# ibejarano/Pynama

Measured on AMD Instinct MI355X. Metric: assembled element-DOFs/sec + CG iterations/sec, 10M-DOF Poisson, 1/2/4/8 MI355X, higher is better.
Workload: dtype f64

## Files before the change

### pynama_amd/csrc/pyn_assemble_lattice.hip

```cpp
#include "pyn_internal.h"
#include "pyn_q1_hex.h"
#include "pyn_lattice.h"

namespace {


__device__ __forceinline__ double lat_affine_inv(const double* __restrict__ S, const double (&E)[3][3], double (&Ji)[3][3]) {
  double J[3][3];
#pragma unroll
  for (int d = 0; d < 3; ++d)
#pragma unroll
    for (int x = 0; x < 3; ++x) J[d][x] = fma(S[d * 3 + 2], E[2][x], fma(S[d * 3 + 1], E[1][x], S[d * 3] * E[0][x]));
  const double c00 = J[1][1] * J[2][2] - J[1][2] * J[2][1];
  const double c01 = J[1][2] * J[2][0] - J[1][0] * J[2][2];
  const double c02 = J[1][0] * J[2][1] - J[1][1] * J[2][0];
  const double det = J[0][0] * c00 + J[0][1] * c01 + J[0][2] * c02;
  const double r = 1.0 / det;
  Ji[0][0] = c00 * r;
  Ji[0][1] = (J[0][2] * J[2][1] - J[0][1] * J[2][2]) * r;
  Ji[0][2] = (J[0][1] * J[1][2] - J[0][2] * J[1][1]) * r;
  Ji[1][0] = c01 * r;
  Ji[1][1] = (J[0][0] * J[2][2] - J[0][2] * J[2][0]) * r;
  Ji[1][2] = (J[0][2] * J[1][0] - J[0][0] * J[1][2]) * r;
  Ji[2][0] = c02 * r;
  Ji[2][1] = (J[0][1] * J[2][0] - J[0][0] * J[2][1]) * r;
  Ji[2][2] = (J[0][0] * J[1][1] - J[0][1] * J[1][0]) * r;
  return det;
}

__device__ __forceinline__ void lat_affine_corners(const LatArgs& T, int n00, int gl, double (&C4)[4][3]) {
  const int nx = T.nx;
  const double* q0 = T.xyz + (int64_t)(lat_plane(T, gl) + n00) * 3;
  const double* qz = T.xyz + (int64_t)(lat_plane(T, gl + 1) + n00) * 3;
  if (T.ablate == 32) {
#pragma unroll
    for (int d = 0; d < 4; ++d)
#pragma unroll
      for (int x = 0; x < 3; ++x) C4[d][x] = (d == x + 1) ? 0.005 : 0.0;
    return;
  }
#pragma unroll
  for (int x = 0; x < 3; ++x) {
    C4[0][x] = q0[x];
    C4[1][x] = q0[3 + x];
    C4[2][x] = q0[3 * nx + x];
    C4[3][x] = qz[x];
  }
}
__device__ __forceinline__ double lat_affine_geom_from(const double* __restrict__ S, const double (&C4)[4][3], double (&Ji)[3][3]) {
  double E[3][3];
#pragma unroll
  for (int d = 0; d < 3; ++d)
#pragma unroll
    for (int x = 0; x < 3; ++x) E[d][x] = C4[d + 1][x] - C4[0][x];
  return lat_affine_inv(S, E, Ji);
}
__device__ __forceinline__ double lat_affine_geom(const LatArgs& T, const double* __restrict__ S, int n00, int gl, double (&Ji)[3][3]) {
  double C4[4][3];
  lat_affine_corners(T, n00, gl, C4);
  return lat_affine_geom_from(S, C4, Ji);
}

__device__ __forceinline__ void lat_affine_L_from(const double (&Ji)[3][3], const double det, double (&L)[36]) {
  double Q[6];
  {
    constexpr int RS[6][2] = {{0, 0}, {1, 1}, {2, 2}, {0, 1}, {0, 2}, {1, 2}};
#pragma unroll
    for (int u = 0; u < 6; ++u) {
      const int a = RS[u][0], b = RS[u][1];
      Q[u] = det * (Ji[0][a] * Ji[0][b] + Ji[1][a] * Ji[1][b] + Ji[2][a] * Ji[2][b]);
    }
  }
  {
    double D[3][3], M[3][2];
#pragma unroll
    for (int u = 0; u < 3; ++u) {
      const double qd = Q[u] * (1.0 / 72.0), qm = Q[3 + u] * (1.0 / 72.0);
      D[u][0] = 4.0 * qd;
      D[u][1] = 8.0 * qd;
      D[u][2] = 16.0 * qd;
      M[u][0] = 12.0 * qm;
      M[u][1] = 24.0 * qm;
    }
    int idx = 0;
#pragma unroll
// ... 687 lines not shown
      unsigned char f[NJ];
#pragma unroll
      for (int j = 0; j < NJ; ++j) {
        const int i = tid + 256 * j;
        const int qx = i % MT::BX, qy = (i / MT::BX) % MT::BY, qz = i / (MT::BX * MT::BY);
        const int x = x0 - 1 + qx, y = y0 - 1 + qy, pl = T.p_own0 + z0 - 1 + qz;
        v[j] = 0.0;
        f[j] = 0;
        if (i < MT::NB && x >= 0 && x < nx && y >= 0 && y < ny && pl >= 0 && pl < T.npl) {
          const int64_t node = lat_plane(T, pl) + y * nx + x;
          f[j] = T.bcmask ? T.bcmask[node] : 0;
          v[j] = xin[node];
        }
      }
#pragma unroll
      for (int j = 0; j < NJ; ++j) {
        const int i = tid + 256 * j;
        if (i < MT::NB) {
          xs[i] = f[j] ? 0.0 : v[j];
          nbc[i] = f[j];
        }
      }
    }
    for (int i = tid; i < MT::NR; i += 256) acc[i] = 0.0;
    __syncthreads();
    {
      const int gx = x0 - 1 + lx, gy = y0 - 1 + ly;
      const bool col_ok = gx >= 0 && gx < nx - 1 && gy >= 0 && gy < ny - 1;
      const int n00 = gy * nx + gx;
      double xb[4], carry[4] = {0.0, 0.0, 0.0, 0.0};
#pragma unroll
      for (int c = 0; c < 4; ++c) xb[c] = xs[boff[c]];
#pragma nounroll
      for (int lz = 0; lz <= TZ; ++lz) {
        const int gl = T.p_own0 + z0 - 1 + lz;
        double xe[8], ye[8];
#pragma unroll
        for (int c = 0; c < 4; ++c) {
          xe[c] = xb[c];
          xe[TOP[c]] = xs[(lz + 1) * (MT::BX * MT::BY) + boff[c]];
        }
        if (col_ok && gl >= 0 && gl < T.npl - 1 && T.ablate != 1) {
          double Ji[3][3];
          const double det = lat_affine_geom(T, S, n00, gl, Ji);
          lat_affine_apply(Ji, det, xe, ye);
        } else {
#pragma unroll
          for (int a = 0; a < 8; ++a) ye[a] = 0.0;
        }
        if (lz >= 1) {
#pragma unroll
          for (int c = 0; c < 4; ++c)
            if (rok[c]) atomicAdd(&acc[(lz - 1) * 225 + roff[c]], carry[c] + ye[c]);
        }
#pragma unroll
        for (int c = 0; c < 4; ++c) {
          carry[c] = ye[TOP[c]];
          xb[c] = xe[TOP[c]];
        }
      }
    }
    __syncthreads();
    for (int s = tid; s < MT::NR; s += 256) {
      const int rx = s % 15, ry = (s / 15) % 15, rz = s / 225;
      const int x = x0 + rx, y = y0 + ry, zo = z0 + rz;
      if (x >= nx || y >= ny || zo >= T.n_own) continue;
      const int64_t node = lat_plane(T, T.p_own0 + zo) + y * nx + x;
      const int bi = ((rz + 1) * MT::BY + ry + 1) * MT::BX + rx + 1;
      const double xv = nbc[bi] ? xin[node] : xs[bi];
      const double yv = nbc[bi] ? xv : acc[s];
      yout[node] = yv;
      if (DOT) dot = fma(yv, xv, dot);
    }
    __syncthreads();
  }
  if (DOT) {
    for (int o = 32; o > 0; o >>= 1) dot += __shfl_xor(dot, o, 64);
    if ((tid & 63) == 0) smd[tid >> 6] = dot;
    __syncthreads();
    if (tid == 0) part[blockIdx.x] = smd[0] + smd[1] + smd[2] + smd[3];
  }
}

struct KleLatArgs {
  LatArgs L;
  double alpha_d, alpha_w;
  const double *wr, *hrsr, *Hr, *hcoor;
  const double* Lel = nullptr;
  int64_t ne = 0;
};

__device__ __forceinline__ double jac_inverse(const double* __restrict__ hc, const double (&X)[8][3], double (&Ji)[3][3]) {
  double J[3][3];
#pragma unroll
  for (int d = 0; d < 3; ++d)
#pragma unroll
    for (int x = 0; x < 3; ++x) {
      double s = 0.0;
#pragma unroll
      for (int c = 0; c < 8; ++c) s = fma(hc[d * 8 + c], X[c][x], s);
      J[d][x] = s;
    }
  const double c00 = J[1][1] * J[2][2] - J[1][2] * J[2][1];
  const double c01 = J[1][2] * J[2][0] - J[1][0] * J[2][2];
  const double c02 = J[1][0] * J[2][1] - J[1][1] * J[2][0];
  const double det = J[0][0] * c00 + J[0][1] * c01 + J[0][2] * c02;
  const double r = 1.0 / det;
  Ji[0][0] = c00 * r;
  Ji[0][1] = (J[0][2] * J[2][1] - J[0][1] * J[2][2]) * r;
  Ji[0][2] = (J[0][1] * J[1][2] - J[0][2] * J[1][1]) * r;
  Ji[1][0] = c01 * r;
  Ji[1][1] = (J[0][0] * J[2][2] - J[0][2] * J[2][0]) * r;
  Ji[1][2] = (J[0][2] * J[1][0] - J[0][0] * J[1][2]) * r;
  Ji[2][0] = c02 * r;
  Ji[2][1] = (J[0][1] * J[2][0] - J[0][0] * J[2][1]) * r;
  Ji[2][2] = (J[0][0] * J[1][1] - J[0][1] * J[1][0]) * r;
  return det;
}

__device__ __forceinline__ void kle_reduced_apply(const KleLatArgs& T, const double (&Ji)[3][3], double det, const double (&xe)[8][3],
                                                  double (&ye)[8][3]) {
  const double* __restrict__ hr = T.hrsr;
  const double cr = T.wr[0] * det;
  const double caw = cr * T.alpha_w, cad = cr * T.alpha_d;
  double Gr[3][8];
#pragma unroll
  for (int d = 0; d < 3; ++d)
#pragma unroll
    for (int a = 0; a < 8; ++a) Gr[d][a] = fma(Ji[d][2], hr[16 + a], fma(Ji[d][1], hr[8 + a], Ji[d][0] * hr[a]));
  double D[3][3];
#pragma unroll
  for (int d = 0; d < 3; ++d)
#pragma unroll
    for (int q = 0; q < 3; ++q) {
      double sacc = 0.0;
#pragma unroll
      for (int b = 0; b < 8; ++b) sacc = fma(Gr[d][b], xe[b][q], sacc);
      D[d][q] = sacc;
    }
  const double tr = cad * (D[0][0] + D[1][1] + D[2][2]);
  double W[3][3];
#pragma unroll
  for (int d = 0; d < 3; ++d)
#pragma unroll
    for (int pp = 0; pp < 3; ++pp) W[d][pp] = d == pp ? tr : caw * (D[d][pp] - D[pp][d]);
#pragma unroll
  for (int a = 0; a < 8; ++a)
#pragma unroll
    for (int pp = 0; pp < 3; ++pp)
      ye[a][pp] = fma(Gr[2][a], W[2][pp], fma(Gr[1][a], W[1][pp], fma(Gr[0][a], W[0][pp], ye[a][pp])));
}

template <int TX, int TY, int TZ, bool AFF, bool DOT>
__global__ void __launch_bounds__(256) lattice_matfree_kle_kernel(KleLatArgs K, const double* __restrict__ xin, double* __restrict__ yout,
                                                                   const int* __restrict__ flag, double* __restrict__ part, int n_tiles) {
  using MT = MfTile<TX, TY, TZ>;
  extern __shared__ __align__(16) double lds[];
  __shared__ double smd[4];
  if (flag && flag[0]) return;
  const LatArgs& T = K.L;
  double* xs = lds;
  double* acc = xs + MT::NB * 3;
  unsigned char* nbc = reinterpret_cast<unsigned char*>(acc + MT::NR * 3);
  const int tid = threadIdx.x;
  const int nx = T.nx, ny = T.ny;
  const double* __restrict__ S = AFF ? T.q.aff + 248 : nullptr;
// ... 911 lines not shown
  }
  PYN_HIP(hipGetLastError());
  return PYN_OK;
}

int pyn_assemble_kle_lattice(pyn_ctx* c, const AsmRequest& rq, const AsmKnobs& k, const AsmPlan& P) {
  KleLatArgs T;
  lat_fill(c, k, T.L);
  kle_fill(c, T, rq.alpha_d, rq.alpha_w);
  T.L.rhs_clean = rq.rhs_clean ? 1 : 0;
  T.L.rcrow = rq.rcrow;
  if (P.kle_general) return launch_kle_lattice<3, 3, 3, true>(c, T, rq.K, rq.Krhs, rq.Rw);
  switch (P.shape) {
    case 1: return launch_kle_lattice<6, 2, 2, false>(c, T, rq.K, rq.Krhs, rq.Rw);
    case 2: return launch_kle_lattice<3, 3, 2, false>(c, T, rq.K, rq.Krhs, rq.Rw);
    case 3: return launch_kle_lattice<4, 3, 3, false>(c, T, rq.K, rq.Krhs, rq.Rw);
    case 4: return launch_kle_lattice<5, 2, 2, false>(c, T, rq.K, rq.Krhs, rq.Rw);
    default: return launch_kle_lattice<3, 3, 3, false>(c, T, rq.K, rq.Krhs, rq.Rw);
  }
}

int pyn_assemble_lattice(pyn_ctx* c, AsmRequest& rq, const AsmKnobs& k, const AsmPlan& P) {
  LatArgs T;
  lat_fill(c, k, T);
  T.A = rq.K;
  T.Arhs = P.krhs_pending ? nullptr : rq.Krhs;
  T.rhs_clean = rq.rhs_clean ? 1 : 0;
  T.rcrow = rq.rcrow;
  T.dinv = P.dinv ? rq.dinv : nullptr;
  rq.dinv_written = T.dinv != nullptr;
  const bool tiles_closed = P.kind == AK_LATTICE && P.k_closed;
  if (tiles_closed && !k.no_lattice_axes && k.lattice_ablate != 32) {
    PYN_TRY(pyn_lattice_axes_ensure(c, k));
    if (c->lat.rect == 1) {
      T.axX = c->lat.d_axes;
      T.axY = T.axX + lat_axis_slots(T.nx);
      T.axZ = T.axY + lat_axis_slots(T.ny);
    }
  }
  PYN_CHECK(!k.lattice_axes_require || T.axX,
            "PYNAMA_LATTICE_AXES_REQUIRE: the axis-table variant of the lattice tile kernel does not apply (%s)",
            !tiles_closed ? "not the parallelepiped tile kernel" : k.no_lattice_axes || k.lattice_ablate == 32 ? "switched off"
                                                                                                              : "mesh not rectilinear");
  int rows_nl = k.lattice_rows_lines == 2 ? 2 : 1;
  while (rows_nl > 1 && lat_rows_lds(T.nx, rows_nl) > 64 * 1024) rows_nl /= 2;
  const char* no_rows = !tiles_closed                                                                ? "not the parallelepiped tile kernel"
                        : k.no_lattice_rows                                                          ? "switched off"
                        : k.lattice_tile >= 0                                                        ? "PYNAMA_LATTICE_TILE asks for a tile shape"
                        : k.lattice_ablate != 0                                                      ? "PYNAMA_LATTICE_ABLATE is set"
                        : k.no_lattice_axes || k.lattice_axes_require || k.no_lattice_tilebc         ? "a switch of the tile kernel's variants is set"
                        : rq.rcrow                                                                   ? "compact Arhs"
                        : c->lat.rect != 1                                                           ? "mesh not rectilinear"
                        : lat_rows_lds(T.nx, rows_nl) > 64 * 1024                                            ? "x-lines too long for the LDS staging"
                                                                                                     : nullptr;
  PYN_CHECK(!k.lattice_rows_require || !no_rows, "PYNAMA_LATTICE_ROWS_REQUIRE: the rows kernel of rectilinear lattices does not apply (%s)",
            no_rows);
  if (!no_rows) {
    if (rows_nl == 2) return launch_lattice_rows<2, 256>(c, T);
    switch (k.lattice_rows_threads) {
      case 128: return launch_lattice_rows<1, 128>(c, T);
      case 512: return launch_lattice_rows<1, 512>(c, T);
      default: return launch_lattice_rows<1, 256>(c, T);
    }
  }
  if (k.lattice_ablate == 64) T.bcmask = nullptr;
  if (P.kind == AK_MARCH) return pyn_assemble_lattice_march(c, k, &T, P.shape);
  const bool affine = P.k_closed, tilebc = !k.no_lattice_tilebc;
  switch (P.shape) {
    case 1: return launch_lattice<7, 7, 7>(c, T, affine, tilebc);
    case 2: return launch_lattice<6, 6, 6>(c, T, affine, tilebc);
    case 3: return launch_lattice<8, 6, 6>(c, T, affine, tilebc);
    case 4: return launch_lattice<7, 6, 6>(c, T, affine, tilebc);
    case 5: return launch_lattice<6, 6, 4>(c, T, affine, tilebc);
    case 6: return launch_lattice<6, 5, 5>(c, T, affine, tilebc);
    case 7: return launch_lattice<7, 4, 4>(c, T, affine, tilebc);
    case 8: return launch_lattice<14, 3, 3>(c, T, affine, tilebc);
    case 9: return launch_lattice<7, 5, 5>(c, T, affine, tilebc);
    default: return launch_lattice<7, 5, 4>(c, T, affine, tilebc);
  }
}


static int mf_select_layers(LatArgs& T, int ntz, int zsel) {
  const int lo = T.p_own0 > 0 ? 1 : 0, hi = T.p_own0 + T.n_own < T.npl ? 1 : 0;
  T.bz0 = 0;
  T.bzs = 1;
  if (zsel == 0) return ntz;
  const int n_int = std::max(0, ntz - lo - hi);
  if (zsel == 1) {
    T.bz0 = lo;
    return n_int;
  }
  if (n_int == 0) return ntz;
  if (lo && hi) {
    T.bzs = ntz - 1;
    return 2;
  }
  T.bz0 = hi ? ntz - 1 : 0;
  return lo + hi;
}

struct MfLaunch {
  int zsel = 0, part_off = 0, max_grid = PYN_MAX_PARTIALS;
  hipStream_t st = nullptr;
};

template <int TX, int TY, int TZ>
static int launch_matfree(pyn_ctx* c, LatArgs& T, bool affine, const double* x, double* y, bool dot, const MfLaunch& L, int* grid_out) {
  using MT = MfTile<TX, TY, TZ>;
  T.ntx = (T.nx + TX - 1) / TX;
  T.nty = (T.ny + TY - 1) / TY;
  const int n_tiles = T.ntx * T.nty * mf_select_layers(T, (T.n_own + TZ - 1) / TZ, L.zsel);
  const int grid = std::min(n_tiles, L.max_grid);
  if (grid_out) *grid_out = grid;
  if (grid == 0) return PYN_OK;
  const int* flag = dot ? c->d_flag : nullptr;
  double* part = dot ? c->d_part + L.part_off : nullptr;
  hipStream_t s = L.st;
  if (affine) {
    if (dot)
      lattice_matfree_laplace_kernel<TX, TY, TZ, true, true><<<grid, 256, MT::BYTES, s>>>(T, x, y, flag, part, n_tiles);
    else
      lattice_matfree_laplace_kernel<TX, TY, TZ, true, false><<<grid, 256, MT::BYTES, s>>>(T, x, y, flag, part, n_tiles);
  } else {
    if (dot)
      lattice_matfree_laplace_kernel<TX, TY, TZ, false, true><<<grid, 256, MT::BYTES, s>>>(T, x, y, flag, part, n_tiles);
    else
      lattice_matfree_laplace_kernel<TX, TY, TZ, false, false><<<grid, 256, MT::BYTES, s>>>(T, x, y, flag, part, n_tiles);
  }
  PYN_HIP(hipGetLastError());
  return PYN_OK;
}

template <int TZ>
static int launch_matfree_march(pyn_ctx* c, LatArgs& T, const double* x, double* y, bool dot, const MfLaunch& L, int* grid_out) {
  using MT = MfTile<15, 15, TZ>;
  T.ntx = (T.nx + 14) / 15;
  T.nty = (T.ny + 14) / 15;
  const int n_tiles = T.ntx * T.nty * mf_select_layers(T, (T.n_own + TZ - 1) / TZ, L.zsel);
  const int grid = std::min(n_tiles, L.max_grid);
  if (grid_out) *grid_out = grid;
  if (grid == 0) return PYN_OK;
  if (dot)
    lattice_matfree_laplace_march_kernel<TZ, true><<<grid, 256, MT::BYTES, L.st>>>(T, x, y, c->d_flag, c->d_part + L.part_off, n_tiles);
  else
    lattice_matfree_laplace_march_kernel<TZ, false><<<grid, 256, MT::BYTES, L.st>>>(T, x, y, nullptr, nullptr, n_tiles);
  PYN_HIP(hipGetLastError());
  return PYN_OK;
}

static bool q1_matfree_supported(const pyn_ctx* c) {
  return c->lat.valid && c->dim == 3 && c->nn == 8 && c->quad[0].ngp == 8;
}

static int matfree_laplace_launch(pyn_ctx* c, const double* x, double* y, bool dot, const MfLaunch& L, int* grid_out) {
  PYN_CHECK(q1_matfree_supported(c), "matrix-free operator: needs a Q1 hexahedral mesh with structured topology and the "
                                               "full-rule tables");
  PYN_CHECK(c->mf_set[PYN_MATFREE_LAPLACE], "matrix-free Laplacian: pyn_matfree_set first");
  LatArgs T;
  int mesh_aff = 0;
  PYN_TRY(lat_fill_args(c, T, &mesh_aff));
  T.bcmask = c->mf_mask[PYN_MATFREE_LAPLACE];
  const bool affine = mesh_aff == 1 && T.q.aff != nullptr && c->aff_standard;
  const char* tl = getenv("PYNAMA_MATFREE_TILE");
  const int sel = tl ? atoi(tl) : (affine ? 6 : 0);
  if (affine && sel >= 6) {
    switch (sel) {
      case 7: return launch_matfree_march<4>(c, T, x, y, dot, L, grid_out);
      case 8: return launch_matfree_march<6>(c, T, x, y, dot, L, grid_out);
      case 9: return launch_matfree_march<12>(c, T, x, y, dot, L, grid_out);
      default: return launch_matfree_march<8>(c, T, x, y, dot, L, grid_out);
    }
  }
  switch (sel) {
    case 1: PYN_TRY((launch_matfree<16, 8, 4>(c, T, affine, x, y, dot, L, grid_out))); break;
    case 2: PYN_TRY((launch_matfree<8, 8, 8>(c, T, affine, x, y, dot, L, grid_out))); break;
    case 3: PYN_TRY((launch_matfree<16, 4, 4>(c, T, affine, x, y, dot, L, grid_out))); break;
    case 4: PYN_TRY((launch_matfree<32, 4, 4>(c, T, affine, x, y, dot, L, grid_out))); break;
    case 5: PYN_TRY((launch_matfree<12, 6, 6>(c, T, affine, x, y, dot, L, grid_out))); break;
    default: PYN_TRY((launch_matfree<16, 8, 8>(c, T, affine, x, y, dot, L, grid_out))); break;
  }
  return PYN_OK;
}

template <int TX, int TY, int TZ>
static int launch_matfree_kle(pyn_ctx* c, KleLatArgs& K, bool affine, const double* x, double* y, bool dot, const MfLaunch& L, int* grid_out) {
  using MT = MfTile<TX, TY, TZ>;
  LatArgs& T = K.L;
  T.ntx = (T.nx + TX - 1) / TX;
  T.nty = (T.ny + TY - 1) / TY;
  const int n_tiles = T.ntx * T.nty * mf_select_layers(T, (T.n_own + TZ - 1) / TZ, L.zsel);
  const int grid = std::min(n_tiles, L.max_grid);
  if (grid_out) *grid_out = grid;
  if (grid == 0) return PYN_OK;
  const size_t lds = (size_t)(MT::NB + MT::NR) * 3 * sizeof(double) + ((MT::NB + 7) & ~7);
  const int* flag = dot ? c->d_flag : nullptr;
  double* part = dot ? c->d_part + L.part_off : nullptr;
  hipStream_t s = L.st;
  if (affine) {
    if (dot)
      lattice_matfree_kle_kernel<TX, TY, TZ, true, true><<<grid, 256, lds, s>>>(K, x, y, flag, part, n_tiles);
    else
      lattice_matfree_kle_kernel<TX, TY, TZ, true, false><<<grid, 256, lds, s>>>(K, x, y, flag, part, n_tiles);
  } else {
    if (dot)
      lattice_matfree_kle_kernel<TX, TY, TZ, false, true><<<grid, 256, lds, s>>>(K, x, y, flag, part, n_tiles);
    else
      lattice_matfree_kle_kernel<TX, TY, TZ, false, false><<<grid, 256, lds, s>>>(K, x, y, flag, part, n_tiles);
  }
  PYN_HIP(hipGetLastError());
  return PYN_OK;
}

static int matfree_kle_launch(pyn_ctx* c, const double* x, double* y, bool dot, const MfLaunch& L, int* grid_out) {
  PYN_CHECK(q1_matfree_supported(c) && c->quad[1].ngp == 1,
            "matrix-free operator: needs a Q1 hexahedral mesh with structured topology and the full- and reduced-rule tables");
  PYN_CHECK(c->mf_set[PYN_MATFREE_KLE], "matrix-free KLE operator: pyn_matfree_set first");
  KleLatArgs K;
  int mesh_aff = 0;
  PYN_TRY(lat_fill_args(c, K.L, &mesh_aff));
  K.L.bcmask = c->mf_mask[PYN_MATFREE_KLE];
  kle_fill(c, K, c->mf_alpha_d[PYN_MATFREE_KLE], c->mf_alpha_w[PYN_MATFREE_KLE]);
  const bool affine = mesh_aff == 1 && K.L.q.aff != nullptr && c->aff_standard;
  const char* tl = getenv("PYNAMA_MATFREE_TILE");
  switch (tl ? atoi(tl) : 0) {
    case 1: PYN_TRY((launch_matfree_kle<16, 8, 4>(c, K, affine, x, y, dot, L, grid_out))); break;
    case 2: PYN_TRY((launch_matfree_kle<6, 6, 6>(c, K, affine, x, y, dot, L, grid_out))); break;
    case 3: PYN_TRY((launch_matfree_kle<16, 4, 4>(c, K, affine, x, y, dot, L, grid_out))); break;
    default: PYN_TRY((launch_matfree_kle<8, 8, 8>(c, K, affine, x, y, dot, L, grid_out))); break;
  }
  return PYN_OK;
}

static int q1_matfree_part(pyn_ctx* c, int op, const double* x, double* y, bool dot, int zsel, int part_off, int max_grid, hipStream_t st,
                           int* grid_out) {
  MfLaunch L;
  L.zsel = zsel;
  L.part_off = part_off;
  L.max_grid = max_grid;
  L.st = st;
  return op == PYN_MATFREE_KLE ? matfree_kle_launch(c, x, y, dot, L, grid_out) : matfree_laplace_launch(c, x, y, dot, L, grid_out);
}

static int q1_matfree_spmv(pyn_ctx* c, int op, const double* x, double* y, bool dot, int* grid_out) {
  return q1_matfree_part(c, op, x, y, dot, 0, 0, PYN_MAX_PARTIALS, c->stream, grid_out);
}

static int q1_matfree_set(pyn_ctx* c, int) {
  PYN_CHECK(q1_matfree_supported(c), "matrix-free operator: needs a Q1 hexahedral mesh with structured topology and the "
                                      "full-rule tables");
  return PYN_OK;
}

static int q1_matfree_bs(const pyn_ctx*, int op) { return op == PYN_MATFREE_KLE ? 3 : 1; }

const MfBackend* pyn_mf_q1() {
  static const MfBackend b = {q1_matfree_supported, q1_matfree_set, q1_matfree_bs, q1_matfree_spmv, q1_matfree_part};
  return &b;
}

int pyn_lattice_symbolic(pyn_ctx* c, bool* done) {
  *done = false;
  const BoxLattice& L = c->box;
  if (!c->lat.valid || !c->lat.std_shape || getenv("PYNAMA_NO_LATTICE_SYMBOLIC")) return PYN_OK;
  LatArgs T;
  T.xyz = c->d_xyz;
  T.rowptr = nullptr;
  T.bcmask = nullptr;
  T.P = L.d_P;
  T.zord = c->lat.d_zord;
  T.nx = L.NX;
  T.ny = L.NY;
  T.npl = L.npl;
  T.p_own0 = L.p_own0;
  T.n_own = L.n_own;
  T.ntx = T.nty = 0;
  T.std_lat = 1;
  T.ablate = 0;
  T.lean = 0;
  T.q = TileArgs();
  T.A = T.Arhs = nullptr;
  const int64_t sx = 3 * (int64_t)L.NX - 2, sy = 3 * (int64_t)L.NY - 2;
  const int64_t nnz = (3 * (int64_t)L.n_own - (L.p_own0 == 0 ? 1 : 0) - (L.p_own0 + L.n_own == L.npl ? 1 : 0)) * sy * sx;
  PYN_CHECK(nnz > 0 && nnz < (int64_t)INT32_MAX, "pattern has %lld entries (int32 CSR limit)", (long long)nnz);
  DevBuf<int32_t> rowptr, colidx;
  PYN_HIP(rowptr.alloc(c->n_owned + 1));
  PYN_HIP(colidx.alloc(nnz));
  lattice_symbolic_kernel<<<(int)((c->n_owned + 1 + 255) / 256), 256, 0, c->stream>>>(T, c->n_owned, rowptr, colidx);
  PYN_HIP(hipGetLastError());
  c->d_rowptr = std::move(rowptr);
  c->d_colidx = std::move(colidx);
  c->nnzb = nnz;
  *done = true;
  return PYN_OK;
}
```

### pynama_amd/csrc/pyn_internal.h

```cpp
#pragma once
#include <hip/hip_runtime.h>
#include <rccl/rccl.h>

#include <algorithm>
#include <atomic>
#include <cstdint>
#include <cstdio>
#include <functional>
#include <map>
#include <memory>
#include <string>
#include <type_traits>
#include <utility>
#include <vector>

#include "../../include/pynama_hip.h"

void pyn_set_error(const char* fmt, ...);

#define PYN_HIP(call)                                                                         \
  do {                                                                                        \
    hipError_t e_ = (call);                                                                   \
    if (e_ != hipSuccess) {                                                                   \
      pyn_set_error("%s:%d %s -> %s", __FILE__, __LINE__, #call, hipGetErrorString(e_));      \
// ... 17 lines not shown
      return PYN_EINVAL;                                                                      \
    }                                                                                         \
  } while (0)

#define PYN_TRY(call)                                                                         \
  do {                                                                                        \
    int rc_ = (call);                                                                         \
    if (rc_ != PYN_OK) return rc_;                                                            \
  } while (0)

inline std::atomic<int64_t> pyn_live_buffers{0}, pyn_live_bytes{0};

template <typename T, bool PINNED = false>
class Buf {
  T* p_ = nullptr;
  size_t n_ = 0;

 public:
  Buf() = default;
  Buf(Buf&& o) noexcept : p_(std::exchange(o.p_, nullptr)), n_(std::exchange(o.n_, 0)) {}
  Buf& operator=(Buf&& o) noexcept {
    if (this != &o) {
      reset();
      p_ = std::exchange(o.p_, nullptr);
      n_ = std::exchange(o.n_, 0);
    }
    return *this;
  }
  ~Buf() { reset(); }
  hipError_t alloc(size_t n) {
    reset();
    if (n == 0) return hipSuccess;
    void* p = nullptr;
    const hipError_t e = PINNED ? hipHostMalloc(&p, n * sizeof(T), hipHostMallocDefault) : hipMalloc(&p, n * sizeof(T));
    if (e != hipSuccess) return e;
    p_ = static_cast<T*>(p);
    n_ = n;
    pyn_live_buffers += 1;
    pyn_live_bytes += (int64_t)(n * sizeof(T));
    return hipSuccess;
  }
  hipError_t grow(size_t n) { return n <= n_ ? hipSuccess : alloc(n); }
  void reset() {
    if (!p_) return;
    (void)(PINNED ? hipHostFree(p_) : hipFree(p_));
    pyn_live_buffers -= 1;
    pyn_live_bytes -= (int64_t)(n_ * sizeof(T));
    p_ = nullptr;
    n_ = 0;
  }
  size_t size() const { return n_; }
  T* get() const { return p_; }
  operator T*() const { return p_; }
};
template <typename T>
using DevBuf = Buf<T, false>;
template <typename T>
using PinBuf = Buf<T, true>;

struct DevTmp : DevBuf<unsigned char> {
  template <typename T>
  T* as() const {
    return reinterpret_cast<T*>(get());
  }
};

template <typename T>
inline int dev_upload(DevBuf<T>& dst, const T* src, size_t n, hipStream_t s) {
  PYN_HIP(dst.alloc(n));
  if (n && src) PYN_HIP(hipMemcpyAsync(dst.get(), src, n * sizeof(T), hipMemcpyHostToDevice, s));
  return PYN_OK;
}

struct QuadTab {
  int ngp = 0;
  DevBuf<double> w;
  DevBuf<double> H;
  DevBuf<double> Hrs;
  DevBuf<double> HrsCoo;
  double wsum = 0.0;
  bool const_grad = false;
};

enum ProductKind { PK_NONE = 0, PK_RAW = 1, PK_SELL = 2, PK_SELLP = 3, PK_SELLB_X = 4, PK_SELLB_D = 5, PK_CSRL = 6, PK_CSRLB = 7, PK_BCSR = 8 };
struct ProductPlan {
  ProductKind kind = PK_NONE;
  int W = 0;
  int lg = 0, unroll = 0;
  size_t lds = 0;
  int wg_cap = -1;
  int max_grid = INT32_MAX;
};

struct MgHier;
struct IbmState;
struct MgHierDelete { void operator()(MgHier* h) const; };
struct IbmStateDelete { void operator()(IbmState* s) const; };

struct DMat {
  int br = 0, bc = 0;
  DevBuf<double> val;
  DevBuf<double> sell_val;
  bool sell_valid = false;
  ProductPlan plan;
  DevBuf<double> dinv;
  bool dinv_valid = false;
  DevBuf<double> lu;
  DevBuf<int> lu_piv;
  int64_t lu_n = 0;
  bool lu_valid = false;
  DevBuf<double> band;
  DevBuf<int> band_perm;
  int64_t band_n = 0, band_kl = 0, band_ku = 0;
  bool band_valid = false;
  std::unique_ptr<MgHier, MgHierDelete> mg;
  bool mg_valid = false;
  int64_t rhs_clean = -2;
  bool rhs_compact = false;
  int64_t c_stamp = -1;
  int64_t c_nr = 0, c_nnzb = 0;
  DevBuf<int32_t> c_crow;
  DevBuf<int32_t> c_rsel;
  DevBuf<int32_t> c_cptr;
  bool live = false;
  void touch() {
    sell_valid = dinv_valid = lu_valid = band_valid = mg_valid = false;
    plan = ProductPlan();
    rhs_clean = -2;
  }
  void release_band() {
    band.reset();
    band_perm.reset();
    band_n = band_kl = band_ku = 0;
    band_valid = false;
  }
  void release_lu() {
    lu.reset();
    lu_piv.reset();
    lu_n = 0;
    lu_valid = false;
    release_band();
  }
};

struct PatchPlan {
  bool user = false;
  DevBuf<int32_t> rowptr, rows, eptr, elem;
  DevBuf<uint4> rowslot4, kmap4;
  int npatch = 0, maxrows = 0, maxlen = 0;
  int64_t npe = 0;
};

struct BoxLattice {
  bool valid = false;
  int dim = 0, ngl = 0;
  int EX = 0, EY = 0, EL = 0;
  int NX = 0, NY = 0;
  int npl = 0, p_own0 = 0, n_own = 0;
  DevBuf<int32_t> d_P;
  std::vector<int32_t> P;
  int64_t plane() const { return (int64_t)NX * NY; }
  int ny() const { return dim == 3 ? NY : npl; }
  int nz() const { return dim == 3 ? npl : 1; }
  bool slab_order() const {
    bool ok = true;
    for (int j = 0; j < npl && ok; ++j) ok = P[j] == (j < p_own0 ? n_own + j : (j >= p_own0 + n_own ? j : j - p_own0)) * plane();
    return ok;
// ... 354 lines not shown
```

### pynama_amd/csrc/pyn_sell.hip

```cpp
#include <hipcub/hipcub.hpp>

#include "pyn_internal.h"

namespace {

constexpr int PAT_MAX = 256;
constexpr int PAT_W = 32;

constexpr int SH = 64;

__global__ void sell_width_kernel(const int32_t* __restrict__ rowptr, int64_t n_rows, int br, int bc, int64_t n_slices,
                                  int* __restrict__ w) {
  for (int64_t s = (int64_t)blockIdx.x * blockDim.x + threadIdx.x; s < n_slices; s += (int64_t)gridDim.x * blockDim.x) {
    int64_t r0 = s * SH, r1 = r0 + SH < n_rows ? r0 + SH : n_rows;
    int m = 0;
    for (int64_t r = r0; r < r1; ++r) {
      const int64_t i = r / br;
      m = max(m, (rowptr[i + 1] - rowptr[i]) * bc);
    }
    w[s] = m;
  }
}

template <bool WITH_COLS>
// ... 1093 lines not shown
                                                            L.A.rhs_compact ? L.A.c_cptr : nullptr);
  return PYN_OK;
}
template <int BR, int BC, bool DOT>
int launch_bcsr(const Launch& L, int* grid) {
  switch (L.P.unroll) {
    case 2: return launch_bcsr_u<BR, BC, 2, DOT>(L, grid);
    case 3: return launch_bcsr_u<BR, BC, 3, DOT>(L, grid);
    case 8: return launch_bcsr_u<BR, BC, 8, DOT>(L, grid);
    default: return launch_bcsr_u<BR, BC, 4, DOT>(L, grid);
  }
}
}

int pyn_sell_spmv_range2(pyn_ctx* c, const DMat& A, const ProductPlan& P, const double* x, double* y, bool dot, int64_t a0, int64_t a1,
                         int64_t b0, int64_t b1, int poff, int max_grid, hipStream_t st, int* grid_out) {
  const SellShape* S = pyn_sell_shape(c, A);
  const int64_t ns = (c->n_owned * A.br + SH - 1) / SH;
  PYN_CHECK(P.kind == PK_RAW || (P.kind != PK_NONE && S), "pyn_sell_ensure first");
  PYN_CHECK(!dot || A.br == A.bc, "fused dot needs a square block shape");
  PYN_CHECK(a0 >= 0 && a0 <= a1 && a1 <= b0 && b0 <= b1 && b1 <= ns, "bad slice ranges");
  const int64_t hb = a1, hl = b0 - a1;
  const int64_t s0 = a0, s1 = b1 - hl;
  if (grid_out) *grid_out = 0;
  if (s0 == s1 && P.kind != PK_RAW) return PYN_OK;
  max_grid = std::min(max_grid, P.max_grid);
  int grid = (int)std::max<int64_t>(1, std::min<int64_t>((s1 - s0 + 3) / 4, max_grid));
  PYN_CHECK(poff + grid <= PYN_MAX_PARTIALS, "partial buffer overflow");
  Launch L{c, A, S, P, x, y, dot ? c->d_flag : nullptr, dot ? c->d_part : nullptr, s0, s1, hb, hl, poff, max_grid, st};
  int p1 = P.W, rc = PYN_OK;
  switch (P.kind) {
    case PK_RAW:
      PYN_CHECK(s0 == 0 && s1 == ns && poff == 0, "32-lane block-CSR product: whole products only");
      rc = dot ? launch_raw<true>(L, &grid) : launch_raw<false>(L, &grid);
      break;
    case PK_SELL:
    case PK_SELLP: rc = dot ? launch_sell<true>(L, grid) : launch_sell<false>(L, grid); break;
    case PK_SELLB_X:
    case PK_SELLB_D:
      p1 = A.bc;
      switch (A.bc) {
        case 1: rc = dot ? launch_sellb<1, true>(L, grid) : launch_sellb<1, false>(L, grid); break;
        case 2: rc = dot ? launch_sellb<2, true>(L, grid) : launch_sellb<2, false>(L, grid); break;
        case 3: rc = dot ? launch_sellb<3, true>(L, grid) : launch_sellb<3, false>(L, grid); break;
        default: rc = dot ? launch_sellb<6, true>(L, grid) : launch_sellb<6, false>(L, grid);
      }
      break;
    case PK_CSRL:
      rc = P.W == 27 ? (dot ? launch_csrl<27, true>(L, &grid) : launch_csrl<27, false>(L, &grid))
                     : (dot ? launch_csrl<32, true>(L, &grid) : launch_csrl<32, false>(L, &grid));
      break;
    case PK_CSRLB:
      rc = P.W == 18   ? (dot ? launch_csrlb<18, true>(L, &grid) : launch_csrlb<18, false>(L, &grid))
           : P.W == 32 ? (dot ? launch_csrlb<32, true>(L, &grid) : launch_csrlb<32, false>(L, &grid))
                       : (dot ? launch_csrlb<50, true>(L, &grid) : launch_csrlb<50, false>(L, &grid));
      break;
    case PK_BCSR: {
      auto node_of = [&](int64_t sl) { return std::min<int64_t>(c->n_owned, sl * SH / A.br); };
      int64_t na0 = node_of(a0), na1 = node_of(a1), nb0 = node_of(b0), nb1 = node_of(b1);
      if (A.rhs_compact) {
        PYN_CHECK(a0 == 0 && b1 == S->ns && a1 == b0 && !dot, "compact imposed-column matrix: whole products only");
        na0 = 0;
        na1 = nb0 = nb1 = A.c_nr;
      }
      L.s0 = na0, L.s1 = nb1 - (nb0 - na1), L.hb = na1, L.hl = nb0 - na1;
      if (L.s0 >= L.s1) return PYN_OK;
      p1 = 1 << P.lg;
      switch (A.br * 8 + A.bc) {
        case 1 * 8 + 1: rc = dot ? launch_bcsr<1, 1, true>(L, &grid) : launch_bcsr<1, 1, false>(L, &grid); break;
        case 2 * 8 + 2: rc = dot ? launch_bcsr<2, 2, true>(L, &grid) : launch_bcsr<2, 2, false>(L, &grid); break;
        case 3 * 8 + 3: rc = dot ? launch_bcsr<3, 3, true>(L, &grid) : launch_bcsr<3, 3, false>(L, &grid); break;
        case 2 * 8 + 1: rc = launch_bcsr<2, 1, false>(L, &grid); break;
        case 3 * 8 + 1: rc = launch_bcsr<3, 1, false>(L, &grid); break;
        case 1 * 8 + 2: rc = launch_bcsr<1, 2, false>(L, &grid); break;
        case 1 * 8 + 3: rc = launch_bcsr<1, 3, false>(L, &grid); break;
        case 3 * 8 + 2: rc = launch_bcsr<3, 2, false>(L, &grid); break;
        case 2 * 8 + 3: rc = launch_bcsr<2, 3, false>(L, &grid); break;
        case 6 * 8 + 3: rc = launch_bcsr<6, 3, false>(L, &grid); break;
        case 3 * 8 + 6: rc = launch_bcsr<3, 6, false>(L, &grid); break;
        default: PYN_CHECK(false, "no block-CSR product for block shape %dx%d", A.br, A.bc);
      }
      break;
    }
    case PK_NONE: break;
  }
  PYN_TRY(rc);
  PYN_HIP(hipGetLastError());
  pyn_product_record(c, P.kind, p1, P.unroll, dot, grid, P.kind == PK_RAW ? 0 : S->maxw);
  if (grid_out) *grid_out = grid;
  return PYN_OK;
}

int pyn_sell_spmv(pyn_ctx* c, const DMat& A, const ProductPlan& P, const double* x, double* y, bool dot, int* grid_out) {
  const int64_t ns = (c->n_owned * A.br + SH - 1) / SH;
  return pyn_sell_spmv_range2(c, A, P, x, y, dot, 0, ns, ns, ns, 0, PYN_MAX_PARTIALS, c->stream, grid_out);
}

void pyn_sell_drop_structure(pyn_ctx* c) {
  c->sell_shapes.clear();
  c->sell_pid.reset();
  c->sell_tab.reset();
  c->sell_npat = 0;
  c->sell_dict_built = false;
}
```

Baseline: 207.1 billion.

## Add separable-axes matrix-free Laplacian kernel for rectilinear affine lattices

Adds a new matrix-free Q1 Laplacian kernel for rectilinear lattices. It applies the operator as a tensor-product sweep using per-axis 1D mass/stiffness coefficient tables (x, y, z), marching through z-chunks with register prefetch of upcoming planes and a shared-memory halo ring. It becomes the default for affine rectilinear meshes and replaces the march kernel, aiming to cut the flops and shared-memory traffic per node compared with the full element-based stencil. The z-chunk size is chosen from an occupancy query. It relies on per-axis tables built at set time and adds two block syncs per plane.

```diff
diff --git a/pynama_amd/csrc/pyn_assemble_lattice.hip b/pynama_amd/csrc/pyn_assemble_lattice.hip
--- a/pynama_amd/csrc/pyn_assemble_lattice.hip
+++ b/pynama_amd/csrc/pyn_assemble_lattice.hip
@@ -1,6 +1,7 @@
 #include "pyn_internal.h"
 #include "pyn_q1_hex.h"
 #include "pyn_lattice.h"
+#include "pyn_matfree_axes.h"
 
 namespace {
 
@@ -854,6 +855,123 @@
   }
 }
 
+template <int TX, int TY, int PF, bool MASK, bool DOT>
+__global__ void __launch_bounds__(256) lattice_matfree_laplace_axes_kernel(LatArgs T, const double* __restrict__ km, int CZ,
+                                                                            const double* __restrict__ xin, double* __restrict__ yout,
+                                                                            const int* __restrict__ flag, double* __restrict__ part,
+                                                                            int n_tiles) {
+  static_assert(TX * TY == 256 && 2 * TY + 2 * (TX + 2) <= 256, "one column per thread, the ring a second one");
+  constexpr int BX = TX + 2, BY = TY + 2, NRING = 2 * TY + 2 * BX;
+  __shared__ double2 mk[BX * BY];
+  __shared__ double2 ab[BX * TY];
+  __shared__ double smd[4];
+  if (flag && flag[0]) return;
+  const int tid = threadIdx.x, nx = T.nx, ny = T.ny;
+  const int lx = tid % TX, ly = tid / TX;
+  const double2* __restrict__ kmp = reinterpret_cast<const double2*>(km);
+  const uint8_t* __restrict__ bc = T.bcmask;
+  int rqx = 0, rqy = 1;
+  const bool ring = tid < NRING, side = tid < 2 * TY;
+  if (ring) mfax_ring_col(tid, TX, TY, rqx, rqy);
+  double dot = 0.0;
+  for (int tb = blockIdx.x; tb < n_tiles; tb += gridDim.x) {
+    const int b = T.ablate == 6 ? tb : xcd_contiguous_tile(tb, n_tiles);
+    int x0, y0, bz, pl0, nz;
+    mfax_tile(b, T.ntx, T.nty, T.bz0, T.bzs, TX, TY, x0, y0, bz);
+    mfax_chunk(T.p_own0, T.n_own, CZ, bz, pl0, nz);
+    const int gx = x0 + lx, gy = y0 + ly, hx = x0 - 1 + rqx, hy = y0 - 1 + rqy;
+    const bool own = gx < nx && gy < ny, rin = ring && hx >= 0 && hx < nx && hy >= 0 && hy < ny;
+    const int cx = mfax_clamp(gx, 0, nx - 1), cy = mfax_clamp(gy, 0, ny - 1), chx = mfax_clamp(hx, 0, nx - 1), chy = mfax_clamp(hy, 0, ny - 1);
+    const int noff = cy * nx + cx, hoff = chy * nx + chx;
+    const double2 X0 = kmp[mfax_km_x(cx, 0)], X1 = kmp[mfax_km_x(cx, 1)], X2 = kmp[mfax_km_x(cx, 2)];
+    const double2 Y0 = kmp[mfax_km_y(nx, cy, 0)], Y1 = kmp[mfax_km_y(nx, cy, 1)], Y2 = kmp[mfax_km_y(nx, cy, 2)];
+    const double2 H0 = kmp[mfax_km_y(nx, chy, 0)], H1 = kmp[mfax_km_y(nx, chy, 1)], H2 = kmp[mfax_km_y(nx, chy, 2)];
+    auto load = [&](int pl, int off, double& v, unsigned char& f) {
+      const int64_t node = (int64_t)lat_plane<true>(T, mfax_plane_clamped(pl, T.npl, pl0, nz)) + off;
+      f = MASK ? bc[node] : 0;
+      v = xin[node];
+    };
+    double rc, hm, hc, qv[PF], hv[PF];
+    unsigned char fc, hf, qf[PF], hqf[PF];
+    load(pl0 - 1, noff, rc, fc);
+    const bool below = mfax_plane_read(pl0 - 1, T.npl, pl0, nz);
+    double pm = (fc || !own || !below) ? 0.0 : rc;
+    load(pl0 - 1, hoff, hc, hf);
+    hm = (hf || !rin || !below) ? 0.0 : hc;
+    load(pl0, noff, rc, fc);
+    load(pl0, hoff, hc, hf);
+    hc = (hf || !rin) ? 0.0 : hc;
+#pragma unroll
+    for (int j = 0; j < PF; ++j) {
+      load(pl0 + 1 + j, noff, qv[j], qf[j]);
+      load(pl0 + 1 + j, hoff, hv[j], hqf[j]);
+    }
+    double2 Zn0 = kmp[mfax_km_z(nx, ny, pl0, 0)], Zn1 = kmp[mfax_km_z(nx, ny, pl0, 1)], Zn2 = kmp[mfax_km_z(nx, ny, pl0, 2)];
+#pragma nounroll
+    for (int lz0 = 0; lz0 < nz; lz0 += PF) {
+#pragma unroll
+      for (int j = 0; j < PF; ++j) {
+        const int lz = lz0 + j, pl = pl0 + lz;
+        if (lz >= nz) break;
+        const bool above = mfax_plane_read(pl + 1, T.npl, pl0, nz);
+        const double rp = qv[j], xp = (qf[j] || !own || !above) ? 0.0 : rp, hp = (hqf[j] || !rin || !above) ? 0.0 : hv[j];
+        const unsigned char fp = qf[j];
+        load(pl + 1 + PF, noff, qv[j], qf[j]);
+        load(pl + 1 + PF, hoff, hv[j], hqf[j]);
+        const double2 Z0 = Zn0, Z1 = Zn1, Z2 = Zn2;
+        const int pz = min(pl + 1, T.npl - 1);
+        Zn0 = kmp[mfax_km_z(nx, ny, pz, 0)];
+        Zn1 = kmp[mfax_km_z(nx, ny, pz, 1)];
+        Zn2 = kmp[mfax_km_z(nx, ny, pz, 2)];
+        const double xc = (fc || !own) ? 0.0 : rc;
+        const double m = fma(Z2.y, xp, fma(Z1.y, xc, Z0.y * pm)), k = fma(Z2.x, xp, fma(Z1.x, xc, Z0.x * pm));
+        mk[(ly + 1) * BX + lx + 1] = make_double2(m, k);
+        double gm = 0.0, gk = 0.0;
+        if (ring) {
+          gm = fma(Z2.y, hp, fma(Z1.y, hc, Z0.y * hm));
+          gk = fma(Z2.x, hp, fma(Z1.x, hc, Z0.x * hm));
+          mk[rqy * BX + rqx] = make_double2(gm, gk);
+        }
+        __syncthreads();
+        double a, bb;
+        {
+          const double2 dn = mk[ly * BX + lx + 1], up = mk[(ly + 2) * BX + lx + 1];
+          a = fma(Y2.y, up.x, fma(Y1.y, m, Y0.y * dn.x));
+          bb = fma(Y2.x, up.x, fma(Y1.x, m, Y0.x * dn.x)) + fma(Y2.y, up.y, fma(Y1.y, k, Y0.y * dn.y));
+          ab[ly * BX + lx + 1] = make_double2(a, bb);
+        }
+        if (side) {
+          const double2 dn = mk[(rqy - 1) * BX + rqx], up = mk[(rqy + 1) * BX + rqx];
+          const double ga = fma(H2.y, up.x, fma(H1.y, gm, H0.y * dn.x));
+          const double gb = fma(H2.x, up.x, fma(H1.x, gm, H0.x * dn.x)) + fma(H2.y, up.y, fma(H1.y, gk, H0.y * dn.y));
+          ab[(rqy - 1) * BX + rqx] = make_double2(ga, gb);
+        }
+        __syncthreads();
+        {
+          const double2 l = ab[ly * BX + lx], r = ab[ly * BX + lx + 2];
+          const double v = fma(X2.x, r.x, fma(X1.x, a, X0.x * l.x)) + fma(X2.y, r.y, fma(X1.y, bb, X0.y * l.y));
+          if (own) {
+            const double yv = fc ? rc : v;
+            yout[(int64_t)lat_plane<true>(T, pl) + noff] = yv;
+            if (DOT) dot = fma(yv, rc, dot);
+          }
+        }
+        pm = xc;
+        rc = rp;
+        fc = fp;
+        hm = hc;
+        hc = hp;
+      }
+    }
+  }
+  if (DOT) {
+    for (int o = 32; o > 0; o >>= 1) dot += __shfl_xor(dot, o, 64);
+    if ((tid & 63) == 0) smd[tid >> 6] = dot;
+    __syncthreads();
+    if (tid == 0) part[blockIdx.x] = smd[0] + smd[1] + smd[2] + smd[3];
+  }
+}
+
 struct KleLatArgs {
   LatArgs L;
   double alpha_d, alpha_w;
@@ -1931,22 +2049,7 @@
 
 
 static int mf_select_layers(LatArgs& T, int ntz, int zsel) {
-  const int lo = T.p_own0 > 0 ? 1 : 0, hi = T.p_own0 + T.n_own < T.npl ? 1 : 0;
-  T.bz0 = 0;
-  T.bzs = 1;
-  if (zsel == 0) return ntz;
-  const int n_int = std::max(0, ntz - lo - hi);
-  if (zsel == 1) {
-    T.bz0 = lo;
-    return n_int;
-  }
-  if (n_int == 0) return ntz;
-  if (lo && hi) {
-    T.bzs = ntz - 1;
-    return 2;
-  }
-  T.bz0 = hi ? ntz - 1 : 0;
-  return lo + hi;
+  return mfax_select_layers(T.npl, T.p_own0, T.n_own, ntz, zsel, T.bz0, T.bzs);
 }
 
 struct MfLaunch {
@@ -1978,6 +2081,7 @@
       lattice_matfree_laplace_kernel<TX, TY, TZ, false, false><<<grid, 256, MT::BYTES, s>>>(T, x, y, flag, part, n_tiles);
   }
   PYN_HIP(hipGetLastError());
+  pyn_product_record(c, PK_MF_TILE, TX, TZ, dot, grid, 0);
   return PYN_OK;
 }
 
@@ -1995,6 +2099,42 @@
   else
     lattice_matfree_laplace_march_kernel<TZ, false><<<grid, 256, MT::BYTES, L.st>>>(T, x, y, nullptr, nullptr, n_tiles);
   PYN_HIP(hipGetLastError());
+  pyn_product_record(c, PK_MF_MARCH, TZ, 0, dot, grid, 0);
+  return PYN_OK;
+}
+
+template <int TX, int TY, int PF>
+static int launch_matfree_axes(pyn_ctx* c, LatArgs& T, int CZ, const double* x, double* y, bool dot, const MfLaunch& L, int* grid_out) {
+  T.ntx = (T.nx + TX - 1) / TX;
+  T.nty = (T.ny + TY - 1) / TY;
+  if (CZ <= 0) {
+    int per_cu = 0;
+    PYN_TRY(pyn_kernel_occupancy(c, reinterpret_cast<const void*>(lattice_matfree_laplace_axes_kernel<TX, TY, PF, true, true>), 256, 0, &per_cu));
+    const int64_t layers = std::max<int64_t>(1, (int64_t)std::max(1, per_cu) * 256 / ((int64_t)T.ntx * T.nty));
+    CZ = (int)std::max<int64_t>(8, (T.n_own + layers - 1) / layers);
+  }
+  const int64_t tiles = (int64_t)T.ntx * T.nty * mf_select_layers(T, (T.n_own + CZ - 1) / CZ, L.zsel);
+  PYN_CHECK(tiles < (int64_t)INT32_MAX, "matrix-free Laplacian: %lld tiles", (long long)tiles);
+  const int n_tiles = (int)tiles;
+  const int grid = std::min(n_tiles, L.max_grid);
+  if (grid_out) *grid_out = grid;
+  if (grid == 0) return PYN_OK;
+  const double* km = c->lat.d_axes.get() + lat_rows_tab_base(T.nx, T.ny, T.npl);
+  const int* flag = dot ? c->d_flag : nullptr;
+  double* part = dot ? c->d_part + L.part_off : nullptr;
+  if (T.bcmask) {
+    if (dot)
+      lattice_matfree_laplace_axes_kernel<TX, TY, PF, true, true><<<grid, 256, 0, L.st>>>(T, km, CZ, x, y, flag, part, n_tiles);
+    else
+      lattice_matfree_laplace_axes_kernel<TX, TY, PF, true, false><<<grid, 256, 0, L.st>>>(T, km, CZ, x, y, flag, part, n_tiles);
+  } else {
+    if (dot)
+      lattice_matfree_laplace_axes_kernel<TX, TY, PF, false, true><<<grid, 256, 0, L.st>>>(T, km, CZ, x, y, flag, part, n_tiles);
+    else
+      lattice_matfree_laplace_axes_kernel<TX, TY, PF, false, false><<<grid, 256, 0, L.st>>>(T, km, CZ, x, y, flag, part, n_tiles);
+  }
+  PYN_HIP(hipGetLastError());
+  pyn_product_record(c, PK_MF_AXES, TX, CZ, dot, grid, 0);
   return PYN_OK;
 }
 
@@ -2013,6 +2153,21 @@
   const bool affine = mesh_aff == 1 && T.q.aff != nullptr && c->aff_standard;
   const char* tl = getenv("PYNAMA_MATFREE_TILE");
   const int sel = tl ? atoi(tl) : (affine ? 6 : 0);
+  if (affine && !tl && c->lat.rect == 1 && c->lat.d_axes && T.std_lat && !getenv("PYNAMA_NO_MATFREE_AXES")) {
+    const char *sh = getenv("PYNAMA_MATFREE_AXES_SHAPE"), *ch = getenv("PYNAMA_MATFREE_AXES_CHUNK"), *pf = getenv("PYNAMA_MATFREE_AXES_PF");
+    const int cz = ch ? atoi(ch) : 0;
+    switch (sh ? atoi(sh) : 0) {
+      case 1: return launch_matfree_axes<64, 4, 2>(c, T, cz, x, y, dot, L, grid_out);
+      case 2: return launch_matfree_axes<16, 16, 2>(c, T, cz, x, y, dot, L, grid_out);
+      default: break;
+    }
+    switch (pf ? atoi(pf) : 0) {
+      case 1: return launch_matfree_axes<32, 8, 1>(c, T, cz, x, y, dot, L, grid_out);
+      case 3: return launch_matfree_axes<32, 8, 3>(c, T, cz, x, y, dot, L, grid_out);
+      case 4: return launch_matfree_axes<32, 8, 4>(c, T, cz, x, y, dot, L, grid_out);
+      default: return launch_matfree_axes<32, 8, 2>(c, T, cz, x, y, dot, L, grid_out);
+    }
+  }
   if (affine && sel >= 6) {
     switch (sel) {
       case 7: return launch_matfree_march<4>(c, T, x, y, dot, L, grid_out);
@@ -2095,9 +2250,14 @@
   return q1_matfree_part(c, op, x, y, dot, 0, 0, PYN_MAX_PARTIALS, c->stream, grid_out);
 }
 
-static int q1_matfree_set(pyn_ctx* c, int) {
+static int q1_matfree_set(pyn_ctx* c, int op) {
   PYN_CHECK(q1_matfree_supported(c), "matrix-free operator: needs a Q1 hexahedral mesh with structured topology and the "
                                       "full-rule tables");
+  if (op == PYN_MATFREE_LAPLACE) {
+    int mesh_aff = 0;
+    PYN_TRY(pyn_mesh_all_affine(c, &mesh_aff));
+    PYN_TRY(pyn_lattice_axes_ensure(c, lat_fill_knobs()));
+  }
   return PYN_OK;
 }
 
diff --git a/pynama_amd/csrc/pyn_internal.h b/pynama_amd/csrc/pyn_internal.h
--- a/pynama_amd/csrc/pyn_internal.h
+++ b/pynama_amd/csrc/pyn_internal.h
@@ -123,7 +123,8 @@
   bool const_grad = false;
 };
 
-enum ProductKind { PK_NONE = 0, PK_RAW = 1, PK_SELL = 2, PK_SELLP = 3, PK_SELLB_X = 4, PK_SELLB_D = 5, PK_CSRL = 6, PK_CSRLB = 7, PK_BCSR = 8 };
+enum ProductKind { PK_NONE = 0, PK_RAW = 1, PK_SELL = 2, PK_SELLP = 3, PK_SELLB_X = 4, PK_SELLB_D = 5, PK_CSRL = 6, PK_CSRLB = 7, PK_BCSR = 8,
+                   PK_MF_TILE = 9, PK_MF_MARCH = 10, PK_MF_AXES = 11 };
 struct ProductPlan {
   ProductKind kind = PK_NONE;
   int W = 0;
diff --git a/pynama_amd/csrc/pyn_matfree_axes.h b/pynama_amd/csrc/pyn_matfree_axes.h
--- /dev/null
+++ b/pynama_amd/csrc/pyn_matfree_axes.h
@@ -0,0 +1,58 @@
+#pragma once
+#include "pyn_lattice_rows.h"
+
+PYN_AX_HD inline int mfax_ring_cols(int TX, int TY) { return 2 * TY + 2 * (TX + 2); }
+
+PYN_AX_HD inline void mfax_ring_col(int h, int TX, int TY, int& qx, int& qy) {
+  const int BX = TX + 2;
+  if (h < 2 * TY) {
+    qy = 1 + (h >> 1);
+    qx = (h & 1) ? TX + 1 : 0;
+  } else {
+    const int hh = h - 2 * TY, top = hh >= BX;
+    qy = top ? TY + 1 : 0;
+    qx = hh - (top ? BX : 0);
+  }
+}
+
+PYN_AX_HD inline int mfax_select_layers(int npl, int p_own0, int n_own, int ntz, int zsel, int& bz0, int& bzs) {
+  const int lo = p_own0 > 0 ? 1 : 0, hi = p_own0 + n_own < npl ? 1 : 0;
+  bz0 = 0;
+  bzs = 1;
+  if (zsel == 0) return ntz;
+  const int n_int = ntz - lo - hi > 0 ? ntz - lo - hi : 0;
+  if (zsel == 1) {
+    bz0 = lo;
+    return n_int;
+  }
+  if (n_int == 0) return ntz;
+  if (lo && hi) {
+    bzs = ntz - 1;
+    return 2;
+  }
+  bz0 = hi ? ntz - 1 : 0;
+  return lo + hi;
+}
+
+PYN_AX_HD inline void mfax_tile(int b, int ntx, int nty, int bz0, int bzs, int TX, int TY, int& x0, int& y0, int& bz) {
+  x0 = (b % ntx) * TX;
+  y0 = ((b / ntx) % nty) * TY;
+  bz = bz0 + (b / (ntx * nty)) * bzs;
+}
+
+PYN_AX_HD inline void mfax_chunk(int p_own0, int n_own, int CZ, int bz, int& pl0, int& nz) {
+  const int z0 = bz * CZ;
+  pl0 = p_own0 + z0;
+  nz = n_own - z0 < CZ ? n_own - z0 : CZ;
+}
+
+PYN_AX_HD inline bool mfax_plane_read(int pl, int npl, int pl0, int nz) { return pl >= 0 && pl < npl && pl >= pl0 - 1 && pl <= pl0 + nz; }
+
+PYN_AX_HD inline int mfax_clamp(int v, int lo, int hi) { return v < lo ? lo : (v > hi ? hi : v); }
+PYN_AX_HD inline int mfax_plane_clamped(int pl, int npl, int pl0, int nz) {
+  return mfax_clamp(pl, pl0 - 1 > 0 ? pl0 - 1 : 0, pl0 + nz < npl - 1 ? pl0 + nz : npl - 1);
+}
+
+PYN_AX_HD inline int mfax_km_x(int x, int d) { return 3 * x + d; }
+PYN_AX_HD inline int mfax_km_y(int nx, int y, int d) { return 3 * (nx + y) + d; }
+PYN_AX_HD inline int mfax_km_z(int nx, int ny, int pl, int d) { return 3 * (nx + ny + pl) + d; }
diff --git a/pynama_amd/csrc/pyn_sell.hip b/pynama_amd/csrc/pyn_sell.hip
--- a/pynama_amd/csrc/pyn_sell.hip
+++ b/pynama_amd/csrc/pyn_sell.hip
@@ -1199,7 +1199,10 @@
       }
       break;
     }
-    case PK_NONE: break;
+    case PK_NONE:
+    case PK_MF_TILE:
+    case PK_MF_MARCH:
+    case PK_MF_AXES: break;
   }
   PYN_TRY(rc);
   PYN_HIP(hipGetLastError());
```

Result: slower. 197.7 billion (-4.5%).
